# liruihui/SP-GAN

Hardware: AMD Instinct MI355X
Metric: G+D train-step shapes/sec @2048 pts, bs=32 per GPU (WGAN-GP) (higher is better)
Workload: dtype f32; 1 GPU; BASELINE configs[1]: Chair-shaped synthetic clouds, 2048 pts, per-GPU batch 32, WGAN + gradient penalty (lambda 10), 1 D-step + 1 G-step, Adam(1e-4, (0.5,0.99)), k=10; one latent per shape (default noise_generator) handed over un-tiled [b,1,128]; global_batch=32, n_points=2048, parallelism=dp1

## Files before the change

### include/spgan_hip.h

```cpp
#ifndef SPGAN_HIP_H
#define SPGAN_HIP_H

#include <stddef.h>
#include <stdint.h>

#ifdef __cplusplus
extern "C" {
#endif

typedef void* spgan_stream_t;

#define SPGAN_OK 0
#define SPGAN_EINVAL (-22)
#define SPGAN_ECOMM (-70)

int spgan_version(void);
const char* spgan_arch(void);


int spgan_knn(const float* x_pm, int B, int N, int C, int k, int mode, int32_t* idx, spgan_stream_t s);

size_t spgan_knn_ws_bytes(int B, int N, int C, int k, int mode);
int spgan_knn_ws(const float* x_pm, int B, int N, int C, int k, int mode, int32_t* idx, void* ws, size_t ws_bytes, spgan_stream_t s);

// ... 48 lines not shown
  int p_group_rows;
  const float* A2; int lda2; const float* p_scale2;
  int a_half, y_bf16;
  int y_half;
  const void* w_image;
  const float* gout_add; int ld_gout_add; const float* gout_scale;
  const float* ad_x; int ad_ldx; long ad_x_shape_stride; int ad_rows;
  const float* ad_mean; const float* ad_var; float ad_eps, ad_slope;
  float* ad_gamma; int ad_ld_gamma, ad_gamma_row0;
} spgan_gemm_nt_args;
int spgan_gemm_nt_y16_ok(const spgan_gemm_nt_args* a);
int spgan_gemm_nt_owns_columns(const spgan_gemm_nt_args* a);
int spgan_gemm_nt_col_blocks(const spgan_gemm_nt_args* a);

int spgan_gemm_nt(const spgan_gemm_nt_args* a, spgan_stream_t s);
size_t spgan_split_bf16x3_image_bytes(int N, int K);
int spgan_split_bf16x3_image(const float* W, int ldw, int N, int K, void* image, spgan_stream_t s);
int spgan_gemm_nt_uses_w_image(const spgan_gemm_nt_args* a);
int spgan_pool_finalize(const float* pool_val, const int32_t* pool_arg, int B, int rows, int C, const float* scale, const float* shift,
                        float slope, float* pooled, int32_t* argmax, float* yarg, spgan_stream_t s);
int spgan_pool_finalize_groups(const float* pool_val, const int32_t* pool_arg, int B, int rows, int C, const float* scale, const float* shift,
                               int group_stride, int shapes_per_group, float slope, float* pooled, int32_t* argmax, float* yarg,
                               int relative_rows, spgan_stream_t s);

typedef struct spgan_gemm_tn_args {
  const float* A; int lda;
  const float* B; int ldb;
  float* C; int ldc;
  int M, Na, Nb;
  int b_mode;
// ... 493 lines not shown
```

### sp-gan_amd/csrc/gemm.hip

```cpp
#include <type_traits>

#include "common.hpp"
#include "adain_epi.hpp"
#include "gemm_wide.hpp"
#include "gemm_tn_wide3.hpp"
#include "sparse_rows.hpp"
#include "split_bf16.hpp"

typedef float f32x16 __attribute__((ext_vector_type(16)));
typedef _Float16 f16x4 __attribute__((ext_vector_type(4)));
typedef _Float16 f16x8 __attribute__((ext_vector_type(8)));
typedef float f32x4v __attribute__((ext_vector_type(4)));

namespace {

constexpr int A_AFFINE_SPARSE = 3;
constexpr int A_AFFINE2 = 4;

constexpr int BM = 128;
constexpr int BK = 32;
constexpr int LDT = BK + 2;

struct Tile {
  int tm, tn;
// ... 7 lines not shown
  r.tn = t % tilesN;
  r.tm = xcd + 8 * (t / tilesN);
  return r;
}

__device__ __forceinline__ float4 ld4(const float* p, bool vec, int k, int K) {
  if (vec && k + 3 < K) return *reinterpret_cast<const float4*>(p);
  float4 v = make_float4(0.f, 0.f, 0.f, 0.f);
  if (k < K) v.x = p[0];
  if (k + 1 < K) v.y = p[1];
  if (k + 2 < K) v.z = p[2];
  if (k + 3 < K) v.w = p[3];
  return v;
}

__device__ __forceinline__ float4 affine_lrelu4(float4 v, float4 sc, float4 sh, float slope) {
  v.x = lrelu_f(fmaf(v.x, sc.x, sh.x), slope);
  v.y = lrelu_f(fmaf(v.y, sc.y, sh.y), slope);
  v.z = lrelu_f(fmaf(v.z, sc.z, sh.z), slope);
  v.w = lrelu_f(fmaf(v.w, sc.w, sh.w), slope);
  return v;
}

__device__ __forceinline__ float4 mask_tail(float4 v, int k, int K) {
  if (k >= K) v.x = 0.f;
  if (k + 1 >= K) v.y = 0.f;
  if (k + 2 >= K) v.z = 0.f;
  if (k + 3 >= K) v.w = 0.f;
  return v;
}

__device__ __forceinline__ int fast_div(int m, int d) {
  int q = (int)((float)m * (1.0f / (float)d));
  q -= (q * d > m) ? 1 : 0;
  q += ((q + 1) * d <= m) ? 1 : 0;
  return q;
}

__device__ __forceinline__ void sparse_add4(float4& v, const float* __restrict__ val, const int32_t* __restrict__ arg, size_t off, int m, int n) {
  if (n > 0 && arg[off] == m) v.x += val[off];
  if (n > 1 && arg[off + 1] == m) v.y += val[off + 1];
  if (n > 2 && arg[off + 2] == m) v.z += val[off + 2];
  if (n > 3 && arg[off + 3] == m) v.w += val[off + 3];
}

__device__ __forceinline__ void st_row4h(float* p, float4 v) {
  f32x4v f = {v.x, v.y, v.z, v.w};
  const f16x4 h = __builtin_convertvector(f, f16x4);
  *reinterpret_cast<f16x4*>(p) = h;
}

typedef __bf16 bf16x4 __attribute__((ext_vector_type(4)));
typedef __bf16 bf16x8 __attribute__((ext_vector_type(8)));
constexpr int LDX3 = 52;

__device__ __forceinline__ void st_row4b3(float* p, float4 v) {
  st_split4(reinterpret_cast<uint32_t*>(p), 16, v);
}

__device__ __forceinline__ void st_row4(float* p, float4 v) {
  *reinterpret_cast<float2*>(p) = make_float2(v.x, v.y);
  *reinterpret_cast<float2*>(p + 2) = make_float2(v.z, v.w);
}

template <int CFG> struct Geo;
template <> struct Geo<0> { static constexpr int WGM = 2, WGN = 2, TI = 2, TJ = 2; };
template <> struct Geo<1> { static constexpr int WGM = 2, WGN = 2, TI = 2, TJ = 1; };
template <> struct Geo<2> { static constexpr int WGM = 4, WGN = 1, TI = 1, TJ = 1; };

template <int CFG>
__device__ __forceinline__ void col_reduce(float (&part)[Geo<CFG>::TJ], float* red, int wm, int wn, int lane) {
  using G = Geo<CFG>;
  constexpr int BN = G::WGN * G::TJ * 32;
#pragma unroll
  for (int j = 0; j < G::TJ; ++j) {
    float v = part[j];
    v += __shfl_xor(v, 32);
// ... 183 lines not shown
      if (AMODE == SPGAN_A_EDGE) peb = ldpar(p.e_bias, k);
      if (AMODE == A_AFFINE2) peb = ldpar(p.p_scale2, k);
    }
#pragma unroll
    for (int i = 0; i < BSLOT; ++i) rb[i] = kok ? ldrow(pW, offW[i], k, vecW) : make_float4(0.f, 0.f, 0.f, 0.f);
  };
  auto sstore = [&](int buf, int k0) {
    float* a = As + buf * BM * LDX;
    float* b = Bs + buf * BN * LDX;
    const int k = k0 + lc4;
    const bool kok = k < p.K;
    if (AMODE != SPGAN_A_PLAIN) {
#pragma unroll
      for (int i = 0; i < 4; ++i) {
        float4 v = ra[i];
        if (AMODE == SPGAN_A_EDGE) {
          v.x = (v.x - ra2[i].x) + peb.x;
          v.y = (v.y - ra2[i].y) + peb.y;
          v.z = (v.z - ra2[i].z) + peb.z;
          v.w = (v.w - ra2[i].w) + peb.w;
        }
        if (AH && AMODE == A_AFFINE2) {
          const float2 rg = make_float2(ra[i].x, ra[i].y), ry = make_float2(ra2[i].x, ra2[i].y);
          const bf16x4 gb = *reinterpret_cast<const bf16x4*>(&rg);
          const f16x4 yh = *reinterpret_cast<const f16x4*>(&ry);
          v = make_float4((float)gb[0], (float)gb[1], (float)gb[2], (float)gb[3]);
          ra2[i] = make_float4((float)yh[0], (float)yh[1], (float)yh[2], (float)yh[3]);
        }
        if (AMODE == A_AFFINE2) {
          v.x = fmaf(v.x, psc.x, fmaf(ra2[i].x, peb.x, psh.x));
          v.y = fmaf(v.y, psc.y, fmaf(ra2[i].y, peb.y, psh.y));
          v.z = fmaf(v.z, psc.z, fmaf(ra2[i].z, peb.z, psh.z));
          v.w = fmaf(v.w, psc.w, fmaf(ra2[i].w, peb.w, psh.w));
        } else
        v = affine_lrelu4(v, psc, psh, p.p_slope);
        if (!FAST) v = mask_tail(v, k, p.K);
// ... 196 lines not shown
        for (int w = 1; w < WGM; ++w) {
          if (pvx[w * BN + q0] > vx) { vx = pvx[w * BN + q0]; ax = pax[w * BN + q0]; }
          if (pvn[w * BN + q0] < vn) { vn = pvn[w * BN + q0]; an = pan[w * BN + q0]; }
        }
        const size_t o = ((size_t)t.tm * Cn + c) * 2;
        p.pool_val[o] = vx; p.pool_val[o + 1] = vn;
        p.pool_arg[o] = ax; p.pool_arg[o + 1] = an;
      }
    }
  } else if (EPI == SPGAN_EPI_LINEAR) {
    float csum[TJ];
    const int rb_g0 = p.rowbias ? fast_div(m0, p.rows_per_group) : 0;
    const bool rb_uniform = p.rowbias && p.rows_per_group > 1 && fast_div(m0 + BM - 1, p.rows_per_group) == rb_g0;
    const bool rb_dense = p.rowbias && p.rows_per_group == 1;
    if (full && (!p.rowbias || rb_uniform || rb_dense)) {
      const float* ab = rb_dense ? p.rowbias + (size_t)rbase * p.ld_rowbias + cbase : nullptr;
      const unsigned lda2 = (unsigned)p.ld_rowbias;
#pragma unroll
      for (int j = 0; j < TJ; ++j) {
        float b = p.bias ? p.bias[cbase + j * 32] : 0.f;
        if (rb_uniform) b += p.rowbias[(size_t)rb_g0 * p.ld_rowbias + cbase + j * 32];
        csum[j] = 0.f;
#pragma unroll
        for (int i = 0; i < TI; ++i) {
          if (ab) {
#pragma unroll
            for (int r = 0; r < 16; ++r) acc[i][j][r] += ab[(size_t)((unsigned)(i * 32 + ROFF(r)) * lda2 + (unsigned)(j * 32))];
          }
#pragma unroll
          for (int r = 0; r < 16; ++r) {
            const float v = acc[i][j][r] + b;
            acc[i][j][r] = v;
            csum[j] += v;
          }
        }
      }
      if (F16 == 1 && pY && p.y_bf16) {
        __bf16* yb = reinterpret_cast<__bf16*>(pY) + (size_t)rbase * p.ldy + cbase;
        const unsigned ldy = (unsigned)p.ldy;
#pragma unroll
        for (int j = 0; j < TJ; ++j)
#pragma unroll
          for (int i = 0; i < TI; ++i)
#pragma unroll
            for (int r = 0; r < 16; ++r) yb[(size_t)((unsigned)(i * 32 + ROFF(r)) * ldy + (unsigned)(j * 32))] = (__bf16)acc[i][j][r];
      } else if (F16 == 1 && pY && p.y_half) {
        _Float16* yb = reinterpret_cast<_Float16*>(pY) + (size_t)rbase * p.ldy + cbase;
        const unsigned ldy = (unsigned)p.ldy;
#pragma unroll
        for (int j = 0; j < TJ; ++j)
#pragma unroll
          for (int i = 0; i < TI; ++i)
#pragma unroll
            for (int r = 0; r < 16; ++r) yb[(size_t)((unsigned)(i * 32 + ROFF(r)) * ldy + (unsigned)(j * 32))] = (_Float16)acc[i][j][r];
      } else if (pY) {
        float* yb = pY + (size_t)rbase * p.ldy + cbase;
        const unsigned ldy = (unsigned)p.ldy;
        auto store_all = [&](auto actf) {
#pragma unroll
          for (int j = 0; j < TJ; ++j)
#pragma unroll
            for (int i = 0; i < TI; ++i)
#pragma unroll
              for (int r = 0; r < 16; ++r) yb[(size_t)((unsigned)(i * 32 + ROFF(r)) * ldy + (unsigned)(j * 32))] = actf(acc[i][j][r]);
        };
        if (p.act == SPGAN_ACT_LRELU) {
          const float sl = p.act_slope;
          store_all([sl](float v) { return lrelu_f(v, sl); });
        } else if (p.act == SPGAN_ACT_TANH) {
          store_all([](float v) { return tanhf(v); });
        } else {
          store_all([](float v) { return v; });
        }
      }
    } else {
#pragma unroll
    for (int j = 0; j < TJ; ++j) {
      const int col = cbase + j * 32;
      const bool cok = col < p.N;
      const float b = (cok && p.bias) ? p.bias[col] : 0.f;
      csum[j] = 0.f;
#pragma unroll
      for (int i = 0; i < TI; ++i)
#pragma unroll
        for (int r = 0; r < 16; ++r) {
          const int row = ROW_OF(i, r);
          float v = acc[i][j][r] + b;
          if (p.rowbias && cok && row < p.M) v += p.rowbias[(size_t)fast_div(row, p.rows_per_group) * p.ld_rowbias + col];
          acc[i][j][r] = v;
          if (row < p.M) csum[j] += v;
          if (cok && row < p.M && pY) {
            float o = v;
            if (p.act == SPGAN_ACT_LRELU) o = lrelu_f(v, p.act_slope);
            else if (p.act == SPGAN_ACT_TANH) o = tanhf(v);
            if (F16 == 1 && p.y_bf16) reinterpret_cast<__bf16*>(pY)[(size_t)row * p.ldy + col] = (__bf16)o;
            else if (F16 == 1 && p.y_half) reinterpret_cast<_Float16*>(pY)[(size_t)row * p.ldy + col] = (_Float16)o;
            else
            pY[(size_t)row * p.ldy + col] = o;
          }
        }
    }
    }
    if (full && (p.stats || p.pool_val)) {
      constexpr int WGM = G::WGM;
      constexpr float NL = (float)(16 * TI);
      float* xs = As;
      float* xm = As + WGM * BN;
      float* xvx = As + 2 * WGM * BN;
      int* xax = reinterpret_cast<int*>(As + 3 * WGM * BN);
      float* xvn = As + 4 * WGM * BN;
      int* xan = reinterpret_cast<int*>(As + 5 * WGM * BN);
      const bool do_pool = p.pool_val != nullptr;
#pragma unroll
      for (int j = 0; j < TJ; ++j) {
        const float sl = csum[j], mean = sl * (1.f / NL);
        float m2 = 0.f;
        float vx = -INFINITY, vn = INFINITY;
        int ax = 0x7fffffff, an = 0x7fffffff;
#pragma unroll
        for (int i = 0; i < TI; ++i)
#pragma unroll
          for (int r = 0; r < 16; ++r) {
            const float v = acc[i][j][r];
            const float d = v - mean;
            m2 = fmaf(d, d, m2);
            if (do_pool) {
              const int row = ROW_OF(i, r);
              if (v > vx) { vx = v; ax = row; }
              if (v < vn) { vn = v; an = row; }
            }
          }
        const float so = __shfl_xor(sl, 32), m2o = __shfl_xor(m2, 32);
        const float dl = (so - sl) * (1.f / NL);
        const float S = sl + so, M2 = (m2 + m2o) + dl * dl * (0.5f * NL);
        if (do_pool) {
          const float ovx = __shfl_xor(vx, 32), ovn = __shfl_xor(vn, 32);
          const int oax = __shfl_xor(ax, 32), oan = __shfl_xor(an, 32);
          if (ovx > vx || (ovx == vx && oax < ax)) { vx = ovx; ax = oax; }
          if (ovn < vn || (ovn == vn && oan < an)) { vn = ovn; an = oan; }
        }
        if (lh == 0) {
          const int c = wm * BN + (wn * TJ + j) * 32 + l31;
          xs[c] = S; xm[c] = M2;
          if (do_pool) { xvx[c] = vx; xax[c] = ax; xvn[c] = vn; xan[c] = an; }
        }
      }
      __syncthreads();
      if (wm == 0 && lh == 0) {
#pragma unroll
        for (int j = 0; j < TJ; ++j) {
          const int c = (wn * TJ + j) * 32 + l31, col = cbase + j * 32;
          float S = xs[c], M2 = xm[c], n = 2.f * NL;
#pragma unroll
          for (int w = 1; w < WGM; ++w) {
            const float Sb = xs[w * BN + c], nb = 2.f * NL;
            const float dl = Sb / nb - S / n;
            M2 = (M2 + xm[w * BN + c]) + dl * dl * (n * nb / (n + nb));
            S += Sb;
            n += nb;
          }
          if (p.stats) {
            float* o = p.stats + ((size_t)t.tm * p.N + col) * 2;
            o[0] = S;
            o[1] = M2;
          }
          if (do_pool) {
            float vx = xvx[c], vn = xvn[c];
            int ax = xax[c], an = xan[c];
#pragma unroll
            for (int w = 1; w < WGM; ++w) {
              if (xvx[w * BN + c] > vx) { vx = xvx[w * BN + c]; ax = xax[w * BN + c]; }
              if (xvn[w * BN + c] < vn) { vn = xvn[w * BN + c]; an = xan[w * BN + c]; }
            }
            const size_t o = ((size_t)t.tm * p.N + col) * 2;
            p.pool_val[o] = vx; p.pool_val[o + 1] = vn;
            p.pool_arg[o] = ax; p.pool_arg[o + 1] = an;
          }
        }
      }
    } else {
    if (p.pool_val) {
      constexpr int WGM = G::WGM;
      float* pvx = pool;
      int* pax = reinterpret_cast<int*>(pool + WGM * BN);
      float* pvn = pool + 2 * WGM * BN;
      int* pan = reinterpret_cast<int*>(pool + 3 * WGM * BN);
#pragma unroll
      for (int j = 0; j < TJ; ++j) {
        float vx = -INFINITY, vn = INFINITY;
        int ax = 0x7fffffff, an = 0x7fffffff;
#pragma unroll
        for (int i = 0; i < TI; ++i)
#pragma unroll
          for (int r = 0; r < 16; ++r) {
// ... 422 lines not shown

inline bool nt_skinny_on(const spgan_gemm_nt_args& a) {
  return a.tile_hint != 1 && a.M > 64 && a.batch <= 1 && !a.tail.enabled && !a.pool_val && !a.sp_val && !a.A2 && !a.a_half && !a.y_bf16 && !a.y_half;
}
inline bool nt_k4_ok(const spgan_gemm_nt_args& a) {
  if (!nt_skinny_on(a) || a.K > 4 || a.a_mode != SPGAN_A_PLAIN || a.N % 4 || a.N < 8 || a.N > 512) return false;
  const int n4 = a.N / 4;
  if (n4 & (n4 - 1)) return false;
  if (a.ldy % 4 || !al16(a.Y)) return false;
  if (a.stats) return false;
  if (a.rowbias && (a.rows_per_group <= 0 || a.rows_per_group % BM || a.M % BM || a.N % 64)) return false;
  if (a.epi_mode == SPGAN_EPI_MASK_OUT) return !a.bias && !a.rowbias && a.ld_ref % 4 == 0 && al16(a.ref);
  return a.epi_mode == SPGAN_EPI_LINEAR;
}

template <int AMODE, int EPI>
int launch_nt(const spgan_gemm_nt_args& a, hipStream_t s) {
  bool fast = (a.K % 4 == 0) && (a.lda % 4 == 0) && (a.ldw % 4 == 0) && al16(a.A) && al16(a.W);
  if (AMODE != SPGAN_A_PLAIN) fast = fast && al16(a.p_scale) && al16(a.p_shift);
  if (AMODE == SPGAN_A_EDGE) fast = fast && al16(a.e_bias);
  if (AMODE == A_AFFINE_SPARSE) fast = fast && al16(a.sp_val) && al16(a.sp_arg);
  if (AMODE == A_AFFINE2) fast = fast && al16(a.A2) && (a.lda2 % 4 == 0) && al16(a.p_scale2);
  if constexpr (AMODE == SPGAN_A_PLAIN && (EPI == SPGAN_EPI_LINEAR || EPI == SPGAN_EPI_MASK_OUT)) {
    if (nt_k4_ok(a)) {
      hipLaunchKernelGGL((gemm_nt_k4_kernel<EPI>), dim3(cdiv(a.M, BM)), dim3(256), 0, s, a, a.N / 4);
      return spgan_launch_status();
    }
  }
  if constexpr (AMODE == A_AFFINE2 && EPI == SPGAN_EPI_EDGE_BNBWD) {
    if (a.a_half) {
      if (a.N > 64 && a.K >= 512) launch_nt_cfg<AMODE, EPI, 0, 1, 1, 1, 1>(a, s);
      else launch_nt_cfg<AMODE, EPI, 1, 0, 1, 1, 1>(a, s);
      return spgan_launch_status();
    }
  }
  if constexpr (AMODE == SPGAN_A_PLAIN && EPI == SPGAN_EPI_LINEAR) {
    if (a.a_half) {
      if (a.N > 64 && a.K >= 512) launch_nt_cfg<AMODE, EPI, 0, 1, 1, 1, 1>(a, s);
      else launch_nt_cfg<AMODE, EPI, 1, 0, 1, 1, 1>(a, s);
      return spgan_launch_status();
    }
// ... 727 lines not shown
  } else {
    if (TB == 128) hipLaunchKernelGGL((gemm_tn_kernel<BMODE, 0, 0>), grid, dim3(256), 0, s, a, rows);
    else if (TB == 64) hipLaunchKernelGGL((gemm_tn_kernel<BMODE, 1, 0>), grid, dim3(256), 0, s, a, rows);
    else hipLaunchKernelGGL((gemm_tn_kernel<BMODE, 2, 0>), grid, dim3(256), 0, s, a, rows);
  }
  if (!a.defer_reduce) launch_reduce(a, splits, s);
  if constexpr (BMODE != SPGAN_A_EDGE) {
    if (a.a_sp_val) hipLaunchKernelGGL((tn_sparse_rows_kernel<BMODE>), dim3(a.Na), dim3(256), 0, s, a);
  }
  return spgan_launch_status();
}

}

static int nt_tile_n(const spgan_gemm_nt_args& a) {
  if (a.a_mode != SPGAN_A_EDGE && !a.A2 && a.epi_mode != SPGAN_EPI_EDGE_BNBWD && spgan_nt_wide16_selected(a)) return spgan_nt_wide16_tile_n(a);
  if (spgan_nt_wide_selected(a)) return 256;
  if (a.a_mode != SPGAN_A_EDGE && !a.A2 && a.epi_mode != SPGAN_EPI_EDGE_BNBWD && spgan_nt_wide3_selected(a)) return spgan_nt_wide3_tile_n(a);
  const bool fast = (a.K % 4 == 0) && (a.lda % 4 == 0) && (a.ldw % 4 == 0) && al16(a.A) && al16(a.W);
  if (a.mfma_f16 == 2 && fast && a.N > 32 && !a.sp_val) return 64;
  if (a.mfma_f16 == 1 && fast && a.N > 32 && !a.sp_val) return (a.N > 64 && a.K >= 512) ? 128 : 64;
  if (a.N > 64 && a.K >= 512) return 128;
  return a.N > 32 ? 64 : 32;
}

extern "C" int spgan_gemm_nt_col_blocks(const spgan_gemm_nt_args* a) {
  if (!a || a->N <= 0) return 0;
  return cdiv(a->N, nt_tile_n(*a));
}

// ... 3 lines not shown
  bool fast = (a->K % 4 == 0) && (a->lda % 4 == 0) && (a->ldw % 4 == 0) && al16(a->A) && al16(a->W);
  if (a->a_mode != SPGAN_A_PLAIN) fast = fast && al16(a->p_scale) && al16(a->p_shift);
  return fast ? 1 : 0;
}

extern "C" int spgan_gemm_nt_y16_ok(const spgan_gemm_nt_args* a) {
  if (!a || a->mfma_f16 != 1 || a->epi_mode != SPGAN_EPI_LINEAR || a->act != SPGAN_ACT_NONE || a->batch > 1 || a->M <= 64 || a->N <= 32) return 0;
  if (a->sp_val) return 0;
  bool fast = (a->K % 4 == 0) && (a->lda % 4 == 0) && (a->ldw % 4 == 0) && al16(a->A) && al16(a->W);
  if (a->a_mode != SPGAN_A_PLAIN) fast = fast && al16(a->p_scale) && al16(a->p_shift);
  if (a->a_mode == SPGAN_A_EDGE) fast = fast && al16(a->e_bias);
  if (a->A2) fast = fast && al16(a->A2) && (a->lda2 % 4 == 0) && al16(a->p_scale2);
  return fast ? 1 : 0;
}

extern "C" int spgan_gemm_nt(const spgan_gemm_nt_args* a, spgan_stream_t s_) {
  hipStream_t s = (hipStream_t)s_;
  SPGAN_CHECK_ARG(a && a->A && a->W && a->M > 0 && a->N > 0 && a->K > 0);
  SPGAN_CHECK_ARG(a->Y || (a->pool_val && a->epi_mode == SPGAN_EPI_LINEAR));
  if (a->pool_val) SPGAN_CHECK_ARG(a->pool_arg && (a->epi_mode == SPGAN_EPI_LINEAR || a->epi_mode == SPGAN_EPI_ADAIN) && a->M > 64);
  SPGAN_CHECK_ARG(a->lda >= a->K && a->ldw >= a->K && a->ldy >= (a->epi_mode == SPGAN_EPI_ADAIN ? a->N / 2 : a->N));
  SPGAN_CHECK_ARG((uint64_t)a->M * (uint64_t)a->lda < (1ull << 32) && (uint64_t)a->N * (uint64_t)a->ldw < (1ull << 32));
  if (a->a_mode != SPGAN_A_PLAIN) SPGAN_CHECK_ARG(a->p_scale && a->p_shift);
  if (a->p_group_rows != 0)
    SPGAN_CHECK_ARG(a->p_group_rows > 0 && a->p_group_rows % BM == 0 && a->M % a->p_group_rows == 0 && a->M > 64);
  if (a->a_mode == SPGAN_A_EDGE) SPGAN_CHECK_ARG(a->e_idx && a->e_bias && a->e_k > 0);
  if (a->rowbias) SPGAN_CHECK_ARG(a->rows_per_group > 0 && a->ld_rowbias >= a->N);
  if (a->sp_val) SPGAN_CHECK_ARG(a->a_mode == SPGAN_A_AFFINE_LRELU && a->sp_arg && a->sp_rows > 0);
  if (a->A2)
    SPGAN_CHECK_ARG(a->a_mode == SPGAN_A_AFFINE_LRELU && !a->sp_val && a->p_scale2 && a->lda2 >= a->K && a->p_group_rows == 0 && a->batch <= 1 &&
                    a->M > 64 && (uint64_t)a->M * (uint64_t)a->lda2 < (1ull << 32) && a->epi_mode != SPGAN_EPI_MASK_OUT);
  if (a->batch > 1)
// ... 166 lines not shown
```

### sp-gan_amd/spgan/_lib.py

```python
from __future__ import annotations

import ctypes as C
import os

_HERE = os.path.dirname(os.path.abspath(__file__))
LIB_PATH = os.path.join(_HERE, "libspgan_hip.so")

c_f32p = C.c_void_p
c_i32p = C.c_void_p
c_i64p = C.c_void_p
stream_t = C.c_void_p


class ColTail(C.Structure):
    _fields_ = [("enabled", C.c_int), ("mode", C.c_int),
                ("out0", c_f32p), ("out1", c_f32p),
                ("gamma", c_f32p), ("beta", c_f32p), ("rmean", c_f32p), ("rvar", c_f32p),
                ("scale", c_f32p), ("shift", c_f32p), ("invstd", c_f32p), ("mean_out", c_f32p),
                ("eps", C.c_float), ("momentum", C.c_float), ("count_rep", C.c_int)]


class GemmNTArgs(C.Structure):
    _fields_ = [
        ("A", c_f32p), ("lda", C.c_int),
# ... 142 lines not shown
SIGNATURES = {
    "spgan_version": (I, []),
    "spgan_arch": (C.c_char_p, []),
    "spgan_knn": (I, [P, I, I, I, I, I, P, P]),
    "spgan_knn_ws_bytes": (SZ, [I, I, I, I, I]),
    "spgan_knn_ws": (I, [P, I, I, I, I, I, P, P, SZ, P]),
    "spgan_csr_build": (I, [P, I, I, I, P, P, P]),
    "spgan_edge_features_cm": (I, [P, P, I, I, I, I, P, P]),
    "spgan_idx_to_local64": (I, [P, I, I, I, P, P]),
    "spgan_idx_from_local64": (I, [P, I, I, I, P, P]),
    "spgan_cm_to_pm": (I, [P, I, I, I, P, P]),
    "spgan_pm_to_cm": (I, [P, I, I, I, P, P]),
    "spgan_concat2": (I, [P, I, P, I, I, P, P]),
    "spgan_gemm_nt": (I, [C.POINTER(GemmNTArgs), P]),
    "spgan_gemm_nt_col_blocks": (I, [C.POINTER(GemmNTArgs)]),
    "spgan_split_bf16x3_image_bytes": (C.c_size_t, [I, I]),
    "spgan_split_bf16x3_image": (I, [P, I, I, I, P, P]),
    "spgan_gemm_nt_uses_w_image": (I, [C.POINTER(GemmNTArgs)]),
    "spgan_gemm_nt_owns_columns": (I, [C.POINTER(GemmNTArgs)]),
    "spgan_pool_finalize": (I, [P, P, I, I, I, P, P, F, P, P, P, P]),
    "spgan_pool_finalize_groups": (I, [P, P, I, I, I, P, P, I, I, F, P, P, P, I, P]),
    "spgan_gemm_tn_ws_bytes": (SZ, [I, I, I]),
    "spgan_gemm_tn_ws_bytes_lp": (SZ, [I, I, I, I]),
    "spgan_gemm_tn_splits_lp": (I, [I, I, I, I]),
    "spgan_gemm_tn": (I, [C.POINTER(GemmTNArgs), P]),
    "spgan_gemm_tn_skinny_multi": (I, [C.POINTER(GemmTNArgs), I, P]),
    "spgan_sparse_rows_nt": (I, [P, P, I, I, I, P, I, I, P, I, P]),
    "spgan_sparse_rows_tn": (I, [P, P, I, I, I, P, I, I, P, P, F, P, I, P]),
    "spgan_affine_act": (I, [P, I, SZ, I, P, P, F, P, P]),
    "spgan_rowscale_outer": (I, [P, I, I, I, P, P, P, P, P, I, I, P]),
# ... 232 lines not shown
```

### sp-gan_amd/spgan/ops.py

```python
from __future__ import annotations

import ctypes as C
import os
from typing import Optional, Tuple

import torch

from . import _lib
from ._lib import GemmDualArgs, GemmNTArgs, GemmTNArgs, check

A_PLAIN, A_AFFINE_LRELU, A_EDGE = 0, 1, 2
EPI_LINEAR, EPI_MASK_OUT, EPI_BNBWD, EPI_EDGE_BNBWD = 0, 1, 2, 3
ACT_NONE, ACT_LRELU, ACT_TANH = 0, 1, 2
BN_EPS, BN_MOMENTUM = 1e-5, 0.1
_BN_MOM = [BN_MOMENTUM]


class bn_momentum:
    def __init__(self, m: float):
        self.m = float(m)

    def __enter__(self):
        self.prev = _BN_MOM[0]
        _BN_MOM[0] = self.m
# ... 93 lines not shown
def _attach_w_image(a, W: Tensor):
    if a.mfma_f16 != 2 or w_image_provider is None or not _lib.load().spgan_gemm_nt_uses_w_image(C.byref(a)):
        return None
    img = w_image_provider(W)
    if img is not None:
        a.w_image = _p(img)
    return img


_NT_TILE_HINT = [0]


class nt_tile_hint:

    def __init__(self, hint: int):
        if hint not in (0, 1, 2):
            raise ValueError("tile_hint must be 0, 1 or 2")
        self.hint = hint

    def __enter__(self):
        self.prev = _NT_TILE_HINT[0]
        _NT_TILE_HINT[0] = self.hint

    def __exit__(self, *exc):
        _NT_TILE_HINT[0] = self.prev


WEIGHTS_EPOCH = [0]
WEIGHTS_EPOCH_OF = {}


def bump_weights_epoch(flat: Tensor) -> None:
    WEIGHTS_EPOCH[0] += 1
    key = flat.untyped_storage().data_ptr()
    WEIGHTS_EPOCH_OF[key] = WEIGHTS_EPOCH_OF.get(key, 0) + 1


def weights_epoch_of(p: Tensor) -> int:
    return WEIGHTS_EPOCH_OF.get(p.untyped_storage().data_ptr(), 0)

# ... 1892 lines not shown
```

Measured before the change: 3626 shapes/s.

## Add persistent streaming NT GEMM kernel with weights resident in LDS

Adds a new persistent-style NT GEMM kernel for K=64/128 linear-epilogue cases. Each workgroup keeps a column block of weights in LDS and streams many row tiles through it. Loading the next tile is double-buffered and overlapped with the current tile's compute and the previous tile's epilogue (bias, activation, stats). This targets repeated weight reloads and per-tile launch and epilogue stalls in the tall-skinny point-cloud GEMMs. The shared epilogue code is moved into a header, and a route-query and tile-count override are exposed for tuning. It is on by default when eligible, and routing could pick this kernel for shapes where the existing wide kernels are faster.

```diff
diff --git a/include/spgan_hip.h b/include/spgan_hip.h
--- a/include/spgan_hip.h
+++ b/include/spgan_hip.h
@@ -86,6 +86,9 @@
 int spgan_gemm_nt_col_blocks(const spgan_gemm_nt_args* a);
 
 int spgan_gemm_nt(const spgan_gemm_nt_args* a, spgan_stream_t s);
+enum { SPGAN_NT_ROUTE_TILES = 0, SPGAN_NT_ROUTE_STREAM = 1 };
+int spgan_gemm_nt_last_route(void);
+void spgan_nt_stream_run_tiles(int tiles);
 size_t spgan_split_bf16x3_image_bytes(int N, int K);
 int spgan_split_bf16x3_image(const float* W, int ldw, int N, int K, void* image, spgan_stream_t s);
 int spgan_gemm_nt_uses_w_image(const spgan_gemm_nt_args* a);
diff --git a/sp-gan_amd/csrc/gemm.hip b/sp-gan_amd/csrc/gemm.hip
--- a/sp-gan_amd/csrc/gemm.hip
+++ b/sp-gan_amd/csrc/gemm.hip
@@ -3,6 +3,8 @@
 #include "common.hpp"
 #include "adain_epi.hpp"
 #include "gemm_wide.hpp"
+#include "gemm_nt_epi.hpp"
+#include "gemm_stream.hpp"
 #include "gemm_tn_wide3.hpp"
 #include "sparse_rows.hpp"
 #include "split_bf16.hpp"
@@ -45,14 +47,6 @@
   return v;
 }
 
-__device__ __forceinline__ float4 affine_lrelu4(float4 v, float4 sc, float4 sh, float slope) {
-  v.x = lrelu_f(fmaf(v.x, sc.x, sh.x), slope);
-  v.y = lrelu_f(fmaf(v.y, sc.y, sh.y), slope);
-  v.z = lrelu_f(fmaf(v.z, sc.z, sh.z), slope);
-  v.w = lrelu_f(fmaf(v.w, sc.w, sh.w), slope);
-  return v;
-}
-
 __device__ __forceinline__ float4 mask_tail(float4 v, int k, int K) {
   if (k >= K) v.x = 0.f;
   if (k + 1 >= K) v.y = 0.f;
@@ -61,13 +55,6 @@
   return v;
 }
 
-__device__ __forceinline__ int fast_div(int m, int d) {
-  int q = (int)((float)m * (1.0f / (float)d));
-  q -= (q * d > m) ? 1 : 0;
-  q += ((q + 1) * d <= m) ? 1 : 0;
-  return q;
-}
-
 __device__ __forceinline__ void sparse_add4(float4& v, const float* __restrict__ val, const int32_t* __restrict__ arg, size_t off, int m, int n) {
   if (n > 0 && arg[off] == m) v.x += val[off];
   if (n > 1 && arg[off + 1] == m) v.y += val[off + 1];
@@ -87,11 +74,6 @@
 
 __device__ __forceinline__ void st_row4b3(float* p, float4 v) {
   st_split4(reinterpret_cast<uint32_t*>(p), 16, v);
-}
-
-__device__ __forceinline__ void st_row4(float* p, float4 v) {
-  *reinterpret_cast<float2*>(p) = make_float2(v.x, v.y);
-  *reinterpret_cast<float2*>(p + 2) = make_float2(v.z, v.w);
 }
 
 template <int CFG> struct Geo;
@@ -305,12 +287,7 @@
 #pragma unroll
       for (int i = 0; i < 4; ++i) {
         float4 v = ra[i];
-        if (AMODE == SPGAN_A_EDGE) {
-          v.x = (v.x - ra2[i].x) + peb.x;
-          v.y = (v.y - ra2[i].y) + peb.y;
-          v.z = (v.z - ra2[i].z) + peb.z;
-          v.w = (v.w - ra2[i].w) + peb.w;
-        }
+        if (AMODE == SPGAN_A_EDGE) v = edge_diff4(v, ra2[i], peb);
         if (AH && AMODE == A_AFFINE2) {
           const float2 rg = make_float2(ra[i].x, ra[i].y), ry = make_float2(ra2[i].x, ra2[i].y);
           const bf16x4 gb = *reinterpret_cast<const bf16x4*>(&rg);
@@ -537,27 +514,7 @@
     const bool rb_uniform = p.rowbias && p.rows_per_group > 1 && fast_div(m0 + BM - 1, p.rows_per_group) == rb_g0;
     const bool rb_dense = p.rowbias && p.rows_per_group == 1;
     if (full && (!p.rowbias || rb_uniform || rb_dense)) {
-      const float* ab = rb_dense ? p.rowbias + (size_t)rbase * p.ld_rowbias + cbase : nullptr;
-      const unsigned lda2 = (unsigned)p.ld_rowbias;
-#pragma unroll
-      for (int j = 0; j < TJ; ++j) {
-        float b = p.bias ? p.bias[cbase + j * 32] : 0.f;
-        if (rb_uniform) b += p.rowbias[(size_t)rb_g0 * p.ld_rowbias + cbase + j * 32];
-        csum[j] = 0.f;
-#pragma unroll
-        for (int i = 0; i < TI; ++i) {
-          if (ab) {
-#pragma unroll
-            for (int r = 0; r < 16; ++r) acc[i][j][r] += ab[(size_t)((unsigned)(i * 32 + ROFF(r)) * lda2 + (unsigned)(j * 32))];
-          }
-#pragma unroll
-          for (int r = 0; r < 16; ++r) {
-            const float v = acc[i][j][r] + b;
-            acc[i][j][r] = v;
-            csum[j] += v;
-          }
-        }
-      }
+      nt_full_bias_csum<TI, TJ>(p, acc, csum, rbase, cbase, rb_g0, rb_uniform, rb_dense);
       if (F16 == 1 && pY && p.y_bf16) {
         __bf16* yb = reinterpret_cast<__bf16*>(pY) + (size_t)rbase * p.ldy + cbase;
         const unsigned ldy = (unsigned)p.ldy;
@@ -577,24 +534,7 @@
 #pragma unroll
             for (int r = 0; r < 16; ++r) yb[(size_t)((unsigned)(i * 32 + ROFF(r)) * ldy + (unsigned)(j * 32))] = (_Float16)acc[i][j][r];
       } else if (pY) {
-        float* yb = pY + (size_t)rbase * p.ldy + cbase;
-        const unsigned ldy = (unsigned)p.ldy;
-        auto store_all = [&](auto actf) {
-#pragma unroll
-          for (int j = 0; j < TJ; ++j)
-#pragma unroll
-            for (int i = 0; i < TI; ++i)
-#pragma unroll
-              for (int r = 0; r < 16; ++r) yb[(size_t)((unsigned)(i * 32 + ROFF(r)) * ldy + (unsigned)(j * 32))] = actf(acc[i][j][r]);
-        };
-        if (p.act == SPGAN_ACT_LRELU) {
-          const float sl = p.act_slope;
-          store_all([sl](float v) { return lrelu_f(v, sl); });
-        } else if (p.act == SPGAN_ACT_TANH) {
-          store_all([](float v) { return tanhf(v); });
-        } else {
-          store_all([](float v) { return v; });
-        }
+        nt_full_store<TI, TJ>(p, pY, acc, rbase, cbase);
       }
     } else {
 #pragma unroll
@@ -625,82 +565,9 @@
     }
     }
     if (full && (p.stats || p.pool_val)) {
-      constexpr int WGM = G::WGM;
-      constexpr float NL = (float)(16 * TI);
-      float* xs = As;
-      float* xm = As + WGM * BN;
-      float* xvx = As + 2 * WGM * BN;
-      int* xax = reinterpret_cast<int*>(As + 3 * WGM * BN);
-      float* xvn = As + 4 * WGM * BN;
-      int* xan = reinterpret_cast<int*>(As + 5 * WGM * BN);
-      const bool do_pool = p.pool_val != nullptr;
-#pragma unroll
-      for (int j = 0; j < TJ; ++j) {
-        const float sl = csum[j], mean = sl * (1.f / NL);
-        float m2 = 0.f;
-        float vx = -INFINITY, vn = INFINITY;
-        int ax = 0x7fffffff, an = 0x7fffffff;
-#pragma unroll
-        for (int i = 0; i < TI; ++i)
-#pragma unroll
-          for (int r = 0; r < 16; ++r) {
-            const float v = acc[i][j][r];
-            const float d = v - mean;
-            m2 = fmaf(d, d, m2);
-            if (do_pool) {
-              const int row = ROW_OF(i, r);
-              if (v > vx) { vx = v; ax = row; }
-              if (v < vn) { vn = v; an = row; }
-            }
-          }
-        const float so = __shfl_xor(sl, 32), m2o = __shfl_xor(m2, 32);
-        const float dl = (so - sl) * (1.f / NL);
-        const float S = sl + so, M2 = (m2 + m2o) + dl * dl * (0.5f * NL);
-        if (do_pool) {
-          const float ovx = __shfl_xor(vx, 32), ovn = __shfl_xor(vn, 32);
-          const int oax = __shfl_xor(ax, 32), oan = __shfl_xor(an, 32);
-          if (ovx > vx || (ovx == vx && oax < ax)) { vx = ovx; ax = oax; }
-          if (ovn < vn || (ovn == vn && oan < an)) { vn = ovn; an = oan; }
-        }
-        if (lh == 0) {
-          const int c = wm * BN + (wn * TJ + j) * 32 + l31;
-          xs[c] = S; xm[c] = M2;
-          if (do_pool) { xvx[c] = vx; xax[c] = ax; xvn[c] = vn; xan[c] = an; }
-        }
-      }
+      nt_records_partial<G::WGM, TI, TJ, BN, true>(p, acc, csum, As, rbase, wm, wn, l31, lh);
       __syncthreads();
-      if (wm == 0 && lh == 0) {
-#pragma unroll
-        for (int j = 0; j < TJ; ++j) {
-          const int c = (wn * TJ + j) * 32 + l31, col = cbase + j * 32;
-          float S = xs[c], M2 = xm[c], n = 2.f * NL;
-#pragma unroll
-          for (int w = 1; w < WGM; ++w) {
-            const float Sb = xs[w * BN + c], nb = 2.f * NL;
-            const float dl = Sb / nb - S / n;
-            M2 = (M2 + xm[w * BN + c]) + dl * dl * (n * nb / (n + nb));
-            S += Sb;
-            n += nb;
-          }
-          if (p.stats) {
-            float* o = p.stats + ((size_t)t.tm * p.N + col) * 2;
-            o[0] = S;
-            o[1] = M2;
-          }
-          if (do_pool) {
-            float vx = xvx[c], vn = xvn[c];
-            int ax = xax[c], an = xan[c];
-#pragma unroll
-            for (int w = 1; w < WGM; ++w) {
-              if (xvx[w * BN + c] > vx) { vx = xvx[w * BN + c]; ax = xax[w * BN + c]; }
-              if (xvn[w * BN + c] < vn) { vn = xvn[w * BN + c]; an = xan[w * BN + c]; }
-            }
-            const size_t o = ((size_t)t.tm * p.N + col) * 2;
-            p.pool_val[o] = vx; p.pool_val[o + 1] = vn;
-            p.pool_arg[o] = ax; p.pool_arg[o + 1] = an;
-          }
-        }
-      }
+      if (wm == 0 && lh == 0) nt_records_merge<G::WGM, TI, TJ, BN, true>(p, As, t.tm, cbase, wn, l31);
     } else {
     if (p.pool_val) {
       constexpr int WGM = G::WGM;
@@ -1153,6 +1020,8 @@
   return a.epi_mode == SPGAN_EPI_LINEAR;
 }
 
+int g_last_route = SPGAN_NT_ROUTE_TILES;
+
 template <int AMODE, int EPI>
 int launch_nt(const spgan_gemm_nt_args& a, hipStream_t s) {
   bool fast = (a.K % 4 == 0) && (a.lda % 4 == 0) && (a.ldw % 4 == 0) && al16(a.A) && al16(a.W);
@@ -1164,6 +1033,12 @@
     if (nt_k4_ok(a)) {
       hipLaunchKernelGGL((gemm_nt_k4_kernel<EPI>), dim3(cdiv(a.M, BM)), dim3(256), 0, s, a, a.N / 4);
       return spgan_launch_status();
+    }
+  }
+  if constexpr (EPI == SPGAN_EPI_LINEAR && (AMODE == SPGAN_A_PLAIN || AMODE == SPGAN_A_AFFINE_LRELU || AMODE == SPGAN_A_EDGE)) {
+    if (spgan_nt_stream_selected(a)) {
+      g_last_route = SPGAN_NT_ROUTE_STREAM;
+      return spgan_launch_nt_stream(a, s);
     }
   }
   if constexpr (AMODE == A_AFFINE2 && EPI == SPGAN_EPI_EDGE_BNBWD) {
@@ -1921,6 +1796,7 @@
 }
 
 static int nt_tile_n(const spgan_gemm_nt_args& a) {
+  if (spgan_nt_stream_selected(a)) return 128;
   if (a.a_mode != SPGAN_A_EDGE && !a.A2 && a.epi_mode != SPGAN_EPI_EDGE_BNBWD && spgan_nt_wide16_selected(a)) return spgan_nt_wide16_tile_n(a);
   if (spgan_nt_wide_selected(a)) return 256;
   if (a.a_mode != SPGAN_A_EDGE && !a.A2 && a.epi_mode != SPGAN_EPI_EDGE_BNBWD && spgan_nt_wide3_selected(a)) return spgan_nt_wide3_tile_n(a);
@@ -1954,8 +1830,11 @@
   return fast ? 1 : 0;
 }
 
+extern "C" int spgan_gemm_nt_last_route(void) { return g_last_route; }
+
 extern "C" int spgan_gemm_nt(const spgan_gemm_nt_args* a, spgan_stream_t s_) {
   hipStream_t s = (hipStream_t)s_;
+  g_last_route = SPGAN_NT_ROUTE_TILES;
   SPGAN_CHECK_ARG(a && a->A && a->W && a->M > 0 && a->N > 0 && a->K > 0);
   SPGAN_CHECK_ARG(a->Y || (a->pool_val && a->epi_mode == SPGAN_EPI_LINEAR));
   if (a->pool_val) SPGAN_CHECK_ARG(a->pool_arg && (a->epi_mode == SPGAN_EPI_LINEAR || a->epi_mode == SPGAN_EPI_ADAIN) && a->M > 64);
diff --git a/sp-gan_amd/csrc/gemm_nt_epi.hpp b/sp-gan_amd/csrc/gemm_nt_epi.hpp
--- /dev/null
+++ b/sp-gan_amd/csrc/gemm_nt_epi.hpp
@@ -0,0 +1,172 @@
+#pragma once
+#include "common.hpp"
+#include "adain_epi.hpp"
+
+#ifndef ROFF
+#define ROFF(r) (((r) & 3) + 8 * ((r) >> 2))
+#endif
+
+__device__ __forceinline__ float4 affine_lrelu4(float4 v, float4 sc, float4 sh, float slope) {
+  v.x = lrelu_f(fmaf(v.x, sc.x, sh.x), slope);
+  v.y = lrelu_f(fmaf(v.y, sc.y, sh.y), slope);
+  v.z = lrelu_f(fmaf(v.z, sc.z, sh.z), slope);
+  v.w = lrelu_f(fmaf(v.w, sc.w, sh.w), slope);
+  return v;
+}
+
+__device__ __forceinline__ float4 edge_diff4(float4 v, float4 c, float4 eb) {
+  v.x = (v.x - c.x) + eb.x;
+  v.y = (v.y - c.y) + eb.y;
+  v.z = (v.z - c.z) + eb.z;
+  v.w = (v.w - c.w) + eb.w;
+  return v;
+}
+
+__device__ __forceinline__ int fast_div(int m, int d) {
+  int q = (int)((float)m * (1.0f / (float)d));
+  q -= (q * d > m) ? 1 : 0;
+  q += ((q + 1) * d <= m) ? 1 : 0;
+  return q;
+}
+
+__device__ __forceinline__ void st_row4(float* p, float4 v) {
+  *reinterpret_cast<float2*>(p) = make_float2(v.x, v.y);
+  *reinterpret_cast<float2*>(p + 2) = make_float2(v.z, v.w);
+}
+
+template <int TI, int TJ>
+__device__ __forceinline__ void nt_full_bias_csum(const spgan_gemm_nt_args& p, f32x16 (&acc)[TI][TJ], float (&csum)[TJ], int rbase, int cbase, int rb_g0,
+                                                  bool rb_uniform, bool rb_dense) {
+  const float* ab = rb_dense ? p.rowbias + (size_t)rbase * p.ld_rowbias + cbase : nullptr;
+  const unsigned lda2 = (unsigned)p.ld_rowbias;
+#pragma unroll
+  for (int j = 0; j < TJ; ++j) {
+    float b = p.bias ? p.bias[cbase + j * 32] : 0.f;
+    if (rb_uniform) b += p.rowbias[(size_t)rb_g0 * p.ld_rowbias + cbase + j * 32];
+    csum[j] = 0.f;
+#pragma unroll
+    for (int i = 0; i < TI; ++i) {
+      if (ab) {
+#pragma unroll
+        for (int r = 0; r < 16; ++r) acc[i][j][r] += ab[(size_t)((unsigned)(i * 32 + ROFF(r)) * lda2 + (unsigned)(j * 32))];
+      }
+#pragma unroll
+      for (int r = 0; r < 16; ++r) {
+        const float v = acc[i][j][r] + b;
+        acc[i][j][r] = v;
+        csum[j] += v;
+      }
+    }
+  }
+}
+
+template <int TI, int TJ>
+__device__ __forceinline__ void nt_full_store(const spgan_gemm_nt_args& p, float* pY, const f32x16 (&acc)[TI][TJ], int rbase, int cbase) {
+  float* yb = pY + (size_t)rbase * p.ldy + cbase;
+  const unsigned ldy = (unsigned)p.ldy;
+  auto store_all = [&](auto actf) {
+#pragma unroll
+    for (int j = 0; j < TJ; ++j)
+#pragma unroll
+      for (int i = 0; i < TI; ++i)
+#pragma unroll
+        for (int r = 0; r < 16; ++r) yb[(size_t)((unsigned)(i * 32 + ROFF(r)) * ldy + (unsigned)(j * 32))] = actf(acc[i][j][r]);
+  };
+  if (p.act == SPGAN_ACT_LRELU) {
+    const float sl = p.act_slope;
+    store_all([sl](float v) { return lrelu_f(v, sl); });
+  } else if (p.act == SPGAN_ACT_TANH) {
+    store_all([](float v) { return tanhf(v); });
+  } else {
+    store_all([](float v) { return v; });
+  }
+}
+
+template <int WGM, int TI, int TJ, int BN, bool POOL>
+__device__ __forceinline__ void nt_records_partial(const spgan_gemm_nt_args& p, const f32x16 (&acc)[TI][TJ], const float (&csum)[TJ], float* x, int rbase, int wm,
+                                                   int wn, int l31, int lh) {
+  constexpr float NL = (float)(16 * TI);
+  float* xs = x;
+  float* xm = x + WGM * BN;
+  float* xvx = x + 2 * WGM * BN;
+  int* xax = reinterpret_cast<int*>(x + 3 * WGM * BN);
+  float* xvn = x + 4 * WGM * BN;
+  int* xan = reinterpret_cast<int*>(x + 5 * WGM * BN);
+  const bool do_pool = POOL && p.pool_val != nullptr;
+#pragma unroll
+  for (int j = 0; j < TJ; ++j) {
+    const float sl = csum[j], mean = sl * (1.f / NL);
+    float m2 = 0.f;
+    float vx = -INFINITY, vn = INFINITY;
+    int ax = 0x7fffffff, an = 0x7fffffff;
+#pragma unroll
+    for (int i = 0; i < TI; ++i)
+#pragma unroll
+      for (int r = 0; r < 16; ++r) {
+        const float v = acc[i][j][r];
+        const float d = v - mean;
+        m2 = fmaf(d, d, m2);
+        if (do_pool) {
+          const int row = rbase + i * 32 + ROFF(r);
+          if (v > vx) { vx = v; ax = row; }
+          if (v < vn) { vn = v; an = row; }
+        }
+      }
+    const float so = __shfl_xor(sl, 32), m2o = __shfl_xor(m2, 32);
+    const float dl = (so - sl) * (1.f / NL);
+    const float S = sl + so, M2 = (m2 + m2o) + dl * dl * (0.5f * NL);
+    if (do_pool) {
+      const float ovx = __shfl_xor(vx, 32), ovn = __shfl_xor(vn, 32);
+      const int oax = __shfl_xor(ax, 32), oan = __shfl_xor(an, 32);
+      if (ovx > vx || (ovx == vx && oax < ax)) { vx = ovx; ax = oax; }
+      if (ovn < vn || (ovn == vn && oan < an)) { vn = ovn; an = oan; }
+    }
+    if (lh == 0) {
+      const int c = wm * BN + (wn * TJ + j) * 32 + l31;
+      xs[c] = S; xm[c] = M2;
+      if (do_pool) { xvx[c] = vx; xax[c] = ax; xvn[c] = vn; xan[c] = an; }
+    }
+  }
+}
+
+template <int WGM, int TI, int TJ, int BN, bool POOL>
+__device__ __forceinline__ void nt_records_merge(const spgan_gemm_nt_args& p, const float* x, int rec, int cbase, int wn, int l31) {
+  constexpr float NL = (float)(16 * TI);
+  const float* xs = x;
+  const float* xm = x + WGM * BN;
+  const float* xvx = x + 2 * WGM * BN;
+  const int* xax = reinterpret_cast<const int*>(x + 3 * WGM * BN);
+  const float* xvn = x + 4 * WGM * BN;
+  const int* xan = reinterpret_cast<const int*>(x + 5 * WGM * BN);
+  const bool do_pool = POOL && p.pool_val != nullptr;
+#pragma unroll
+  for (int j = 0; j < TJ; ++j) {
+    const int c = (wn * TJ + j) * 32 + l31, col = cbase + j * 32;
+    float S = xs[c], M2 = xm[c], n = 2.f * NL;
+#pragma unroll
+    for (int w = 1; w < WGM; ++w) {
+      const float Sb = xs[w * BN + c], nb = 2.f * NL;
+      const float dl = Sb / nb - S / n;
+      M2 = (M2 + xm[w * BN + c]) + dl * dl * (n * nb / (n + nb));
+      S += Sb;
+      n += nb;
+    }
+    if (p.stats) {
+      float* o = p.stats + ((size_t)rec * p.N + col) * 2;
+      o[0] = S;
+      o[1] = M2;
+    }
+    if (do_pool) {
+      float vx = xvx[c], vn = xvn[c];
+      int ax = xax[c], an = xan[c];
+#pragma unroll
+      for (int w = 1; w < WGM; ++w) {
+        if (xvx[w * BN + c] > vx) { vx = xvx[w * BN + c]; ax = xax[w * BN + c]; }
+        if (xvn[w * BN + c] < vn) { vn = xvn[w * BN + c]; an = xan[w * BN + c]; }
+      }
+      const size_t o = ((size_t)rec * p.N + col) * 2;
+      p.pool_val[o] = vx; p.pool_val[o + 1] = vn;
+      p.pool_arg[o] = ax; p.pool_arg[o + 1] = an;
+    }
+  }
+}
diff --git a/sp-gan_amd/csrc/gemm_stream.hip b/sp-gan_amd/csrc/gemm_stream.hip
--- /dev/null
+++ b/sp-gan_amd/csrc/gemm_stream.hip
@@ -0,0 +1,236 @@
+#include <atomic>
+#include <cstdlib>
+#include <type_traits>
+
+#include "gemm_nt_epi.hpp"
+#include "gemm_stream.hpp"
+#include "gemm_wide.hpp"
+
+namespace {
+
+constexpr int SM = 128, SN = 128;
+constexpr int STHREADS = 512;
+constexpr int WGM = 2, WGN = 4, TI = 2, TJ = 1;
+constexpr int CK = 64, LDC = CK + 2;
+constexpr int RPP = STHREADS / (CK / 4);
+constexpr int AS = SM / RPP;
+constexpr int XW = 2 * WGM * SN;
+constexpr int SLOTS = 256;
+constexpr int MIN_RUN = 4;
+
+template <int K> constexpr size_t stream_lds() { return (size_t)(SN * (K + 2) + 2 * SM * LDC + 2 * XW) * sizeof(float); }
+
+template <int AMODE, int K>
+__global__ __launch_bounds__(STHREADS, 1) void gemm_nt_stream_kernel(const spgan_gemm_nt_args p_, int tpw, int wgs_per_cb) {
+  const spgan_gemm_nt_args& p = p_;
+  constexpr bool affine = AMODE != SPGAN_A_PLAIN;
+  constexpr bool edge = AMODE == SPGAN_A_EDGE;
+  constexpr int LDW = K + 2;
+  constexpr int NCH = K / CK;
+  constexpr int KK = CK / 4;
+  static_assert(NCH == 1 || NCH == 2, "K = 64 or 128");
+  static_assert(!edge || NCH == 1, "the per-edge operand's index pipeline is per tile");
+  extern __shared__ __attribute__((aligned(16))) float smem[];
+  float* Ws = smem;
+  float* As = smem + SN * LDW;
+  float* X = As + 2 * SM * LDC;
+
+  const int ncb = p.N / SN;
+  const int per_xcd = gridDim.x >> 3;
+  const int L = (blockIdx.x & 7) * per_xcd + (blockIdx.x >> 3);
+  if (L >= wgs_per_cb * ncb) return;
+  const int wg = L / ncb, cb = L - wg * ncb;
+  const int tilesM = p.M / SM;
+  const int t0 = wg * tpw, t1 = min(tilesM, t0 + tpw);
+  if (t0 >= t1) return;
+  const int n0 = cb * SN;
+  const int tid = threadIdx.x, lane = tid & 63, wave = tid >> 6, wm = wave / WGN, wn = wave % WGN;
+  const int l31 = lane & 31, lh = lane >> 5;
+  const int lrow = tid >> 4, lc4 = (tid & 15) * 4;
+  const int cbase = n0 + wn * (TJ * 32) + l31;
+
+#pragma unroll
+  for (int c = 0; c < NCH; ++c) {
+    float4 rw[AS];
+#pragma unroll
+    for (int i = 0; i < AS; ++i) rw[i] = *reinterpret_cast<const float4*>(p.W + (size_t)(n0 + lrow + RPP * i) * p.ldw + c * CK + lc4);
+#pragma unroll
+    for (int i = 0; i < AS; ++i) st_row4(Ws + (lrow + RPP * i) * LDW + c * CK + lc4, rw[i]);
+  }
+
+  float4 ra[AS];
+  float4 rc[edge ? AS : 1];
+  int nidx[edge ? AS : 1];
+  float4 psc = make_float4(1.f, 1.f, 1.f, 1.f), psh = make_float4(0.f, 0.f, 0.f, 0.f), peb = psh;
+  if (edge) peb = *reinterpret_cast<const float4*>(p.e_bias + lc4);
+  const unsigned ulda = (unsigned)p.lda;
+
+  auto iload = [&](int t) {
+#pragma unroll
+    for (int i = 0; i < AS; ++i) nidx[edge ? i : 0] = p.e_idx[t * SM + lrow + RPP * i];
+  };
+  auto gload = [&](int t, int kc) {
+    const int m0 = t * SM;
+    const unsigned k = (unsigned)(kc * CK + lc4);
+    if (edge) {
+#pragma unroll
+      for (int i = 0; i < AS; ++i) {
+        ra[i] = *reinterpret_cast<const float4*>(p.A + ((unsigned)nidx[edge ? i : 0] * ulda + k));
+        rc[edge ? i : 0] = *reinterpret_cast<const float4*>(p.A + ((unsigned)fast_div(m0 + lrow + RPP * i, p.e_k) * ulda + k));
+      }
+    } else {
+      const unsigned oa = (unsigned)(m0 + lrow) * ulda + k;
+#pragma unroll
+      for (int i = 0; i < AS; ++i) ra[i] = *reinterpret_cast<const float4*>(p.A + (oa + (unsigned)(RPP * i) * ulda));
+    }
+    if (affine) {
+      const int g = p.p_group_rows > 0 ? fast_div(m0, p.p_group_rows) : 0;
+      psc = *reinterpret_cast<const float4*>(p.p_scale + (size_t)g * K + k);
+      psh = *reinterpret_cast<const float4*>(p.p_shift + (size_t)g * K + k);
+    }
+  };
+  auto sstore = [&](int buf) {
+    float* a = As + buf * SM * LDC + lrow * LDC + lc4;
+#pragma unroll
+    for (int i = 0; i < AS; ++i) {
+      float4 v = ra[i];
+      if (edge) v = edge_diff4(v, rc[edge ? i : 0], peb);
+      if (affine) v = affine_lrelu4(v, psc, psh, p.p_slope);
+      st_row4(a + RPP * i * LDC, v);
+    }
+  };
+  auto compute = [&](int buf, int kc, f32x16 (&acc)[TI][TJ]) {
+    const float* a = As + buf * SM * LDC + (wm * TI * 32 + l31) * LDC + 2 * lh;
+    const float* b = Ws + (wn * TJ * 32 + l31) * LDW + kc * CK + 2 * lh;
+#pragma unroll
+    for (int kk = 0; kk < KK; ++kk) {
+      float2 af[TI];
+#pragma unroll
+      for (int i = 0; i < TI; ++i) af[i] = *reinterpret_cast<const float2*>(a + i * 32 * LDC + kk * 4);
+      const float2 bf = *reinterpret_cast<const float2*>(b + kk * 4);
+#pragma unroll
+      for (int i = 0; i < TI; ++i) acc[i][0] = __builtin_amdgcn_mfma_f32_32x32x2f32(af[i].x, bf.x, acc[i][0], 0, 0, 0);
+#pragma unroll
+      for (int i = 0; i < TI; ++i) acc[i][0] = __builtin_amdgcn_mfma_f32_32x32x2f32(af[i].y, bf.y, acc[i][0], 0, 0, 0);
+    }
+  };
+  auto epi_a = [&](int t, f32x16 (&acc)[TI][TJ], int xb) {
+    const int rbase = t * SM + wm * TI * 32 + 4 * lh;
+    float csum[TJ];
+    nt_full_bias_csum<TI, TJ>(p, acc, csum, rbase, cbase, 0, false, false);
+    if (p.Y) nt_full_store<TI, TJ>(p, p.Y, acc, rbase, cbase);
+    if (p.stats) nt_records_partial<WGM, TI, TJ, SN, false>(p, acc, csum, X + xb * XW, rbase, wm, wn, l31, lh);
+  };
+  auto epi_b = [&](int t, int xb) {
+    if (p.stats && wm == 0 && lh == 0) nt_records_merge<WGM, TI, TJ, SN, false>(p, X + xb * XW, t, cbase, wn, l31);
+  };
+  auto step = [&](int t, int par, f32x16 (&cur)[TI][TJ], f32x16 (&prev)[TI][TJ]) {
+#pragma unroll
+    for (int i = 0; i < TI; ++i)
+#pragma unroll
+      for (int r = 0; r < 16; ++r) cur[i][0][r] = 0.f;
+#pragma unroll
+    for (int kc = 0; kc < NCH; ++kc) {
+      const int buf = NCH == 1 ? par : kc;
+      const bool in_tile = kc + 1 < NCH;
+      const bool more = in_tile || t + 1 < t1;
+      if (more) {
+        gload(in_tile ? t : t + 1, in_tile ? kc + 1 : 0);
+        if (edge && t + 2 < t1) iload(t + 2);
+      }
+      compute(buf, kc, cur);
+      if (kc == 0 && t > t0) epi_a(t - 1, prev, par ^ 1);
+      if (more) sstore(buf ^ 1);
+      __syncthreads();
+      if (kc == 0 && t > t0) epi_b(t - 1, par ^ 1);
+    }
+  };
+  auto last = [&](int t, int par, f32x16 (&cur)[TI][TJ]) {
+    epi_a(t, cur, par);
+    __syncthreads();
+    epi_b(t, par);
+  };
+
+  if (edge) iload(t0);
+  gload(t0, 0);
+  if (edge && t0 + 1 < t1) iload(t0 + 1);
+  sstore(0);
+  __syncthreads();
+  f32x16 acc0[TI][TJ], acc1[TI][TJ];
+  for (int t = t0;;) {
+    step(t, 0, acc0, acc1);
+    if (++t >= t1) {
+      last(t - 1, 0, acc0);
+      break;
+    }
+    step(t, 1, acc1, acc0);
+    if (++t >= t1) {
+      last(t - 1, 1, acc1);
+      break;
+    }
+  }
+}
+
+std::atomic<int> g_run_tiles{0};
+
+inline bool al16(const void* q) { return (reinterpret_cast<uintptr_t>(q) & 15) == 0; }
+
+void stream_plan(int M, int N, int* tpw, int* wgs_per_cb) {
+  const int ncb = N / SN, tilesM = M / SM;
+  int w = SLOTS / ncb;
+  if (w < 1) w = 1;
+  int t = cdiv(tilesM, w);
+  const int forced = g_run_tiles.load(std::memory_order_relaxed);
+  if (forced > 0) t = forced;
+  *tpw = t;
+  *wgs_per_cb = cdiv(tilesM, t);
+}
+
+template <int AMODE, int K>
+int launch(const spgan_gemm_nt_args& a, hipStream_t s) {
+  constexpr size_t lds = stream_lds<K>();
+  static LdsOptIn opt;
+  opt.ensure(reinterpret_cast<const void*>(&gemm_nt_stream_kernel<AMODE, K>), (int)lds);
+  int tpw, wgs_per_cb;
+  stream_plan(a.M, a.N, &tpw, &wgs_per_cb);
+  const int grid = cdiv((long)wgs_per_cb * (a.N / SN), 8) * 8;
+  hipLaunchKernelGGL((gemm_nt_stream_kernel<AMODE, K>), dim3(grid), dim3(STHREADS), lds, s, a, tpw, wgs_per_cb);
+  return spgan_launch_status();
+}
+
+template <int AMODE>
+int launch_k(const spgan_gemm_nt_args& a, hipStream_t s) {
+  return a.K == 64 ? launch<AMODE, 64>(a, s) : launch<AMODE, 128>(a, s);
+}
+
+}
+
+bool spgan_nt_stream_eligible(const spgan_gemm_nt_args& a) {
+  if (a.mfma_f16 != 0 || a.epi_mode != SPGAN_EPI_LINEAR) return false;
+  if (a.M < SM || a.M % SM || a.N % SN || (a.K != 64 && a.K != 128) || a.M >= (1 << 24)) return false;
+  if (a.batch > 1 || a.tail.enabled || a.rowbias || a.pool_val || a.sp_val || a.A2 || a.a_half || a.y_bf16 || a.y_half || !a.Y) return false;
+  if (a.lda % 4 || a.ldw % 4 || !al16(a.A) || !al16(a.W)) return false;
+  if (a.a_mode == SPGAN_A_PLAIN) return true;
+  if (!al16(a.p_scale) || !al16(a.p_shift)) return false;
+  if (a.a_mode == SPGAN_A_AFFINE_LRELU) return true;
+  return a.a_mode == SPGAN_A_EDGE && a.K == 64 && a.p_group_rows == 0 && al16(a.e_bias);
+}
+
+bool spgan_nt_stream_selected(const spgan_gemm_nt_args& a) {
+  static const bool off = getenv("SPGAN_NT_STREAM") && atoi(getenv("SPGAN_NT_STREAM")) == 0;
+  if (off || (a.tile_hint != 0 && a.tile_hint != 3) || !spgan_nt_stream_eligible(a)) return false;
+  if (a.tile_hint == 3) return true;
+  if (a.stats && spgan_nt_wide_selected(a)) return false;
+  const int rows = a.p_group_rows > 0 ? a.p_group_rows : a.M;
+  const int ncb = a.N / SN;
+  const int w = SLOTS / ncb < 1 ? 1 : SLOTS / ncb;
+  return cdiv(rows / SM, w) >= MIN_RUN;
+}
+
+int spgan_launch_nt_stream(const spgan_gemm_nt_args& a, hipStream_t s) {
+  if (a.a_mode == SPGAN_A_PLAIN) return launch_k<SPGAN_A_PLAIN>(a, s);
+  if (a.a_mode == SPGAN_A_AFFINE_LRELU) return launch_k<SPGAN_A_AFFINE_LRELU>(a, s);
+  return launch<SPGAN_A_EDGE, 64>(a, s);
+}
+
+extern "C" void spgan_nt_stream_run_tiles(int tiles) { g_run_tiles.store(tiles > 0 ? tiles : 0, std::memory_order_relaxed); }
diff --git a/sp-gan_amd/csrc/gemm_stream.hpp b/sp-gan_amd/csrc/gemm_stream.hpp
--- /dev/null
+++ b/sp-gan_amd/csrc/gemm_stream.hpp
@@ -0,0 +1,6 @@
+#pragma once
+#include "common.hpp"
+
+bool spgan_nt_stream_eligible(const spgan_gemm_nt_args& a);
+bool spgan_nt_stream_selected(const spgan_gemm_nt_args& a);
+int spgan_launch_nt_stream(const spgan_gemm_nt_args& a, hipStream_t s);
diff --git a/sp-gan_amd/spgan/_lib.py b/sp-gan_amd/spgan/_lib.py
--- a/sp-gan_amd/spgan/_lib.py
+++ b/sp-gan_amd/spgan/_lib.py
@@ -180,6 +180,8 @@
     "spgan_concat2": (I, [P, I, P, I, I, P, P]),
     "spgan_gemm_nt": (I, [C.POINTER(GemmNTArgs), P]),
     "spgan_gemm_nt_col_blocks": (I, [C.POINTER(GemmNTArgs)]),
+    "spgan_gemm_nt_last_route": (I, []),
+    "spgan_nt_stream_run_tiles": (None, [I]),
     "spgan_split_bf16x3_image_bytes": (C.c_size_t, [I, I]),
     "spgan_split_bf16x3_image": (I, [P, I, I, I, P, P]),
     "spgan_gemm_nt_uses_w_image": (I, [C.POINTER(GemmNTArgs)]),
diff --git a/sp-gan_amd/spgan/ops.py b/sp-gan_amd/spgan/ops.py
--- a/sp-gan_amd/spgan/ops.py
+++ b/sp-gan_amd/spgan/ops.py
@@ -131,8 +131,8 @@
 class nt_tile_hint:
 
     def __init__(self, hint: int):
-        if hint not in (0, 1, 2):
-            raise ValueError("tile_hint must be 0, 1 or 2")
+        if hint not in (0, 1, 2, 3):
+            raise ValueError("tile_hint must be 0, 1, 2 or 3")
         self.hint = hint
 
     def __enter__(self):
@@ -141,6 +141,14 @@
 
     def __exit__(self, *exc):
         _NT_TILE_HINT[0] = self.prev
+
+
+def _nt_last_route() -> int:
+    return int(_lib.load().spgan_gemm_nt_last_route())
+
+
+def _nt_stream_run_tiles(tiles: int) -> None:
+    _lib.load().spgan_nt_stream_run_tiles(int(tiles))
 
 
 WEIGHTS_EPOCH = [0]
```

After: 3647 shapes/s, median of 6. No clear change (+0.6%).
